# Snowdar/asv-subtools

Measured on AMD Instinct MI355X. Metric: utterances/sec (200-frame) embedding extraction + EER, 1/2/4/8 MI355X, higher is better.
Workload: dtype bf16; 1 GPU; BASELINE configs[1]: standard TDNN x-vector: Xvector(80,10,training=False), 80-dim fbank, 256 utterances x 200 frames per GPU per step, features resident in HBM, f32 embeddings out; global_batch_utts=256, frames_per_utt=200, parallelism=utterance shards x1, streams=2

## Files before the change

asv-subtools_amd/csrc/kernels_tdnn_p8.hip:

```cpp
#include <algorithm>
#include <cstdlib>
#include <type_traits>

#define ASV_GLDS_CLOBBER_M0
#include "lds_dma.h"

namespace asv {
namespace {

constexpr int P8_HALF = 128 * 128;
constexpr int P8_OFF_B0 = 0, P8_OFF_A0 = P8_HALF, P8_OFF_B1 = 2 * P8_HALF, P8_OFF_A1 = 3 * P8_HALF;
constexpr int P8_BUF = 4 * P8_HALF;
constexpr int P8_PARAM_OFF = 2 * P8_BUF;
constexpr int P8_LDS_BYTES = 2 * P8_BUF + 3 * 256 * 4;
constexpr int P8_ROWB = 128;

template <int ET, int VAR, bool ONE_TAP, int PH>
__global__ __launch_bounds__(512, 2) void tdnn_gemm_p8_kernel(const TdnnKernelParams p, int m_tiles, int n_tiles) {
  static_assert(PH == 2 || PH == 4, "phases per K-tile");
  constexpr bool STAGGER = !(VAR == 1 || VAR == 3), PRIO = !(VAR == 2 || VAR == 3), SKELETON = VAR == 4;
  constexpr bool NO_DMA = SKELETON || VAR == 5, NO_READS = SKELETON || VAR == 6;
  auto stamp = [&](int k) {
    if constexpr (VAR == 7) {
      if (threadIdx.x == 0) reinterpret_cast<unsigned long long *>(p.partial)[(size_t)blockIdx.x * 8 + k] = __builtin_amdgcn_s_memtime();
    }
  };
  stamp(0);
  __shared__ __attribute__((aligned(16))) unsigned char lds[P8_LDS_BYTES];
  const int tid = threadIdx.x, lane = tid & 63;
  const int wave = __builtin_amdgcn_readfirstlane(tid >> 6);
  const int wm = wave >> 2, wn = wave & 3;
  const int lr = lane & 31, lh = lane >> 5;

  const int tile = xcd_swizzle(blockIdx.x, m_tiles * n_tiles);
  const int m0 = (tile / n_tiles) * 256;
  const int n0 = (tile % n_tiles) * 256;

  const unsigned char *xg = reinterpret_cast<const unsigned char *>(p.x);
  const unsigned char *wg = reinterpret_cast<const unsigned char *>(p.w);
  const uint32_t x_pitch = (uint32_t)p.ldx * 2u;
  const int cin_pad = p.cin_pad;
  const int n_taps = ONE_TAP ? 1 : p.n_taps;
  const uint32_t w_pitch = (uint32_t)n_taps * (uint32_t)cin_pad * 2u;
  const uint32_t lds_base = __builtin_amdgcn_readfirstlane((uint32_t)(uintptr_t)(lds_byte *)lds);
  const int nkt = (cin_pad / 64) * n_taps;

  float *lds_par = reinterpret_cast<float *>(lds + P8_PARAM_OFF);
  auto stage_params = [&]() {
    if (wave < 3) {
      const float *src = (wave == 0) ? p.bias : (wave == 1 ? p.scale : p.shift);
      if (src != nullptr) {
        glds16_s_m0(src + n0, (uint32_t)lane * 16u, __builtin_amdgcn_readfirstlane(lds_base + (uint32_t)P8_PARAM_OFF + (uint32_t)wave * 1024u));
      } else {
        const float dflt = (wave == 1) ? 1.0f : 0.0f;
        *reinterpret_cast<float4 *>(lds_par + wave * 256 + lane * 4) = make_float4(dflt, dflt, dflt, dflt);
      }
    }
  };

  const int g_row = lane >> 3, g_slot = lane & 7;
  int a_row[2];
  uint32_t a_slot[2];
  uint32_t a_voff[2][2];
  uint32_t b_off[2];
  const int last_row = p.rows - 1;
#pragma unroll
  for (int i = 0; i < 2; ++i) {
    const int r = (wave * 2 + i) * 8 + g_row;
    const uint32_t slot16 = (uint32_t)(g_slot ^ ((r >> 1) & 7)) * 16u;
    a_row[i] = m0 + (r >> 6) * 128 + (r & 63);
    a_slot[i] = slot16;
    a_voff[0][i] = (uint32_t)a_row[i] * x_pitch + slot16;
    a_voff[1][i] = (uint32_t)min(a_row[i] + 64, last_row) * x_pitch + slot16;
    b_off[i] = (uint32_t)(n0 + (r >> 5) * 64 + (r & 31)) * w_pitch + slot16;
  }
  int v_taps = p.taps[0];
  if (!ONE_TAP) {
#pragma unroll
    for (int t = 1; t < ASV_MAX_TAPS; ++t) v_taps = (lane == t) ? p.taps[t] : v_taps;
  }

  auto stage = [&](int which, int c, int t, int b, bool in_loop) {
    if (NO_DMA && in_loop) return;
    const uint32_t dst0 = lds_base + (uint32_t)b * P8_BUF + (uint32_t)which * P8_HALF + (uint32_t)wave * 2048u;
    if (which & 1) {
      const unsigned char *base = xg + (size_t)c * 128;
      if (ONE_TAP) {
#pragma unroll
        for (int i = 0; i < 2; ++i) glds16_s_m0(base, a_voff[which == 3][i], __builtin_amdgcn_readfirstlane(dst0 + i * 1024u));
      } else {
        const int d = __builtin_amdgcn_readlane(v_taps, t) + (which == 3 ? 64 : 0);
#pragma unroll
        for (int i = 0; i < 2; ++i) {
          const int row = min(max(a_row[i] + d, 0), last_row);
          glds16_s_m0(base, (uint32_t)row * x_pitch + a_slot[i], __builtin_amdgcn_readfirstlane(dst0 + i * 1024u));
        }
      }
    } else {
      const unsigned char *base = wg + ((size_t)t * cin_pad + (size_t)c * 64) * 2 + (which == 2 ? (size_t)32 * w_pitch : 0);
#pragma unroll
      for (int i = 0; i < 2; ++i) glds16_s_m0(base, b_off[i], __builtin_amdgcn_readfirstlane(dst0 + i * 1024u));
    }
  };

  const uint32_t sw = (uint32_t)((lr >> 1) & 7);
  const uint32_t a_base = (uint32_t)(wm * 64 + lr) * P8_ROWB, b_base = (uint32_t)(wn * 32 + lr) * P8_ROWB;
  uint32_t a_addr[4], b_addr[4];
#pragma unroll
  for (int kg = 0; kg < 4; ++kg) {
    const uint32_t s16 = (((uint32_t)(kg * 2 + lh)) ^ sw) * 16u;
    a_addr[kg] = a_base + s16;
    b_addr[kg] = b_base + s16;
  }

  f32x16_t acc[4][2];
#pragma unroll
  for (int i = 0; i < 4; ++i)
#pragma unroll
    for (int j = 0; j < 2; ++j)
#pragma unroll
      for (int r = 0; r < 16; ++r) acc[i][j][r] = 0.0f;

  if constexpr (PH == 2) {
    stage_params();
    stage(0, 0, 0, 0, false); stage(1, 0, 0, 0, false); stage(2, 0, 0, 0, false); stage(3, 0, 0, 0, false);
    {
      int c1 = 0, t1 = 1;
      if (t1 == n_taps) { t1 = 0; c1 = 1; }
      if (nkt > 1) {
        stage(0, c1, t1, 1, false); stage(1, c1, t1, 1, false);
        asm volatile("s_waitcnt vmcnt(4)" ::: "memory");
      } else {
        asm volatile("s_waitcnt vmcnt(0)" ::: "memory");
      }
    }
    __builtin_amdgcn_s_barrier();
    asm volatile("" ::: "memory");
    uint4 wb0[4], wb1[4], xa[2][4];
    if (NO_READS) {
#pragma unroll
      for (int kg = 0; kg < 4; ++kg) {
        wb0[kg] = make_uint4(lane, 1, 2, 3); wb1[kg] = make_uint4(3, lane, 1, 0);
        xa[0][kg] = make_uint4(1, 1, lane, 1); xa[1][kg] = make_uint4(2, 2, 2, lane);
      }
    }
    stamp(1);
    if (STAGGER && wm == 1) __builtin_amdgcn_s_barrier();
    auto mma_q = [&](const uint4 (&wfr)[4], int j, int i0) {
#pragma unroll
      for (int kg = 0; kg < 4; ++kg)
#pragma unroll
        for (int i2 = 0; i2 < 2; ++i2) acc[i0 + i2][j] = mfma16<ET>(wfr[kg], xa[i2][kg], acc[i0 + i2][j]);
    };
    auto barrier = [&]() {
      __builtin_amdgcn_s_barrier();
      asm volatile("" ::: "memory");
    };
    int c1 = 0, t1 = 0, c2 = 0, t2 = 0;
    auto adv = [&](int &c, int &t) { if (++t == n_taps) { t = 0; ++c; } };
    adv(c1, t1); adv(c2, t2); adv(c2, t2);
    auto ktile2 = [&](int kt, auto tail_c) {
      constexpr int TAIL = decltype(tail_c)::value;
      const int b = kt & 1;
      const unsigned char *L = lds + (uint32_t)b * P8_BUF;
      if (!NO_READS) {
#pragma unroll
        for (int kg = 0; kg < 4; ++kg) wb0[kg] = *reinterpret_cast<const uint4 *>(L + P8_OFF_B0 + b_addr[kg]);
#pragma unroll
        for (int kg = 0; kg < 4; ++kg)
#pragma unroll
          for (int i2 = 0; i2 < 2; ++i2) xa[i2][kg] = *reinterpret_cast<const uint4 *>(L + P8_OFF_A0 + i2 * (32 * P8_ROWB) + a_addr[kg]);
#pragma unroll
        for (int kg = 0; kg < 4; ++kg) wb1[kg] = *reinterpret_cast<const uint4 *>(L + P8_OFF_B1 + b_addr[kg]);
        __builtin_amdgcn_sched_barrier(0);
      }
      if (TAIL <= 1) { stage(2, c1, t1, b ^ 1, true); stage(3, c1, t1, b ^ 1, true); }
      if (TAIL <= 1) asm volatile("s_waitcnt vmcnt(8) lgkmcnt(0)" ::: "memory");
      else asm volatile("s_waitcnt vmcnt(0) lgkmcnt(0)" ::: "memory");
      barrier();
      __builtin_amdgcn_sched_barrier(0);
      if (PRIO) __builtin_amdgcn_s_setprio(1);
      mma_q(wb0, 0, 0);
      mma_q(wb1, 1, 0);
      if (PRIO) __builtin_amdgcn_s_setprio(0);
      __builtin_amdgcn_sched_barrier(0);
      barrier();
      if (!NO_READS) {
#pragma unroll
        for (int kg = 0; kg < 4; ++kg)
#pragma unroll
          for (int i2 = 0; i2 < 2; ++i2) xa[i2][kg] = *reinterpret_cast<const uint4 *>(L + P8_OFF_A1 + i2 * (32 * P8_ROWB) + a_addr[kg]);
        __builtin_amdgcn_sched_barrier(0);
      }
      if (TAIL == 0) { stage(0, c2, t2, b, true); stage(1, c2, t2, b, true); }
      if (TAIL == 0) asm volatile("s_waitcnt vmcnt(6) lgkmcnt(0)" ::: "memory");
      else if (TAIL == 1) asm volatile("s_waitcnt vmcnt(2) lgkmcnt(0)" ::: "memory");
      else asm volatile("s_waitcnt lgkmcnt(0)" ::: "memory");
      barrier();
      __builtin_amdgcn_sched_barrier(0);
      if (PRIO) __builtin_amdgcn_s_setprio(1);
      mma_q(wb1, 1, 2);
      mma_q(wb0, 0, 2);
      if (PRIO) __builtin_amdgcn_s_setprio(0);
      __builtin_amdgcn_sched_barrier(0);
      barrier();
      adv(c1, t1); adv(c2, t2);
    };
    using J0 = std::integral_constant<int, 0>; using J1 = std::integral_constant<int, 1>; using J2 = std::integral_constant<int, 2>;
    int kt = 0;
    for (; kt + 2 < nkt; ++kt) ktile2(kt, J0{});
    if (kt + 1 < nkt) { ktile2(kt, J1{}); ++kt; }
    ktile2(kt, J2{});
  } else {
  {
    int c1 = 0, t1 = 1;
    if (t1 == n_taps) { t1 = 0; c1 = 1; }
    stage_params();
    stage(0, 0, 0, 0, false); stage(1, 0, 0, 0, false); stage(2, 0, 0, 0, false); stage(3, 0, 0, 0, false);
    if (nkt > 1) {
      stage(0, c1, t1, 1, false); stage(1, c1, t1, 1, false); stage(2, c1, t1, 1, false);
      asm volatile("s_waitcnt vmcnt(6)" ::: "memory");
    } else {
      asm volatile("s_waitcnt vmcnt(0)" ::: "memory");
    }
  }
  __builtin_amdgcn_s_barrier();
  asm volatile("" ::: "memory");

  uint4 wb0[2][4], wb1[4], xa[2][4];
  if (NO_READS) {
#pragma unroll
    for (int kg = 0; kg < 4; ++kg) {
      wb0[0][kg] = make_uint4(lane, 1, 2, 3); wb0[1][kg] = make_uint4(lane, 5, 2, 3); wb1[kg] = make_uint4(3, lane, 1, 0);
      xa[0][kg] = make_uint4(1, 1, lane, 1); xa[1][kg] = make_uint4(2, 2, 2, lane);
    }
  } else {
#pragma unroll
    for (int kg = 0; kg < 4; ++kg) wb0[0][kg] = *reinterpret_cast<const uint4 *>(lds + P8_OFF_B0 + b_addr[kg]);
  }
  if (STAGGER && wm == 1) __builtin_amdgcn_s_barrier();

  auto mma_q = [&](const uint4 (&wfr)[4], int j, int i0) {
    if (PRIO) __builtin_amdgcn_s_setprio(1);
#pragma unroll
    for (int kg = 0; kg < 4; ++kg)
#pragma unroll
      for (int i2 = 0; i2 < 2; ++i2) acc[i0 + i2][j] = mfma16<ET>(wfr[kg], xa[i2][kg], acc[i0 + i2][j]);
    if (PRIO) __builtin_amdgcn_s_setprio(0);
  };
  auto barrier = [&]() {
    __builtin_amdgcn_s_barrier();
    asm volatile("" ::: "memory");
  };

  int cs = 0, ts = 0;
  auto advance = [&]() { if (++ts == n_taps) { ts = 0; ++cs; } };
  advance();
  auto ktile = [&](auto tail_c, auto par_c) {
    constexpr int TAIL = decltype(tail_c)::value, PAR = decltype(par_c)::value;
    const unsigned char *L = lds + PAR * P8_BUF, *Ln = lds + (PAR ^ 1) * P8_BUF;
    if (!NO_READS) {
#pragma unroll
      for (int kg = 0; kg < 4; ++kg)
#pragma unroll
        for (int i2 = 0; i2 < 2; ++i2) xa[i2][kg] = *reinterpret_cast<const uint4 *>(L + P8_OFF_A0 + i2 * (32 * P8_ROWB) + a_addr[kg]);
      __builtin_amdgcn_sched_barrier(0);
    }
    if (TAIL <= 1) stage(3, cs, ts, PAR ^ 1, true);
    if (TAIL == 0) advance();
    barrier();
    asm volatile("s_waitcnt lgkmcnt(0)" ::: "memory");
    __builtin_amdgcn_sched_barrier(0);
    mma_q(wb0[PAR], 0, 0);
    __builtin_amdgcn_sched_barrier(0);
    barrier();
    if (!NO_READS) {
#pragma unroll
      for (int kg = 0; kg < 4; ++kg) wb1[kg] = *reinterpret_cast<const uint4 *>(L + P8_OFF_B1 + b_addr[kg]);
      __builtin_amdgcn_sched_barrier(0);
    }
    if (TAIL == 0) stage(0, cs, ts, PAR, true);
    barrier();
    asm volatile("s_waitcnt lgkmcnt(0)" ::: "memory");
    __builtin_amdgcn_sched_barrier(0);
    mma_q(wb1, 1, 0);
    __builtin_amdgcn_sched_barrier(0);
    barrier();
    if (!NO_READS) {
#pragma unroll
      for (int kg = 0; kg < 4; ++kg)
#pragma unroll
        for (int i2 = 0; i2 < 2; ++i2) xa[i2][kg] = *reinterpret_cast<const uint4 *>(L + P8_OFF_A1 + i2 * (32 * P8_ROWB) + a_addr[kg]);
      __builtin_amdgcn_sched_barrier(0);
    }
    if (TAIL == 0) {
      stage(1, cs, ts, PAR, true);
      asm volatile("s_waitcnt vmcnt(10)" ::: "memory");
    } else if (TAIL == 1) {
      asm volatile("s_waitcnt vmcnt(6)" ::: "memory");
    }
    barrier();
    asm volatile("s_waitcnt lgkmcnt(0)" ::: "memory");
    __builtin_amdgcn_sched_barrier(0);
    mma_q(wb1, 1, 2);
    __builtin_amdgcn_sched_barrier(0);
    barrier();
    if (!NO_READS && TAIL <= 1) {
#pragma unroll
      for (int kg = 0; kg < 4; ++kg) wb0[PAR ^ 1][kg] = *reinterpret_cast<const uint4 *>(Ln + P8_OFF_B0 + b_addr[kg]);
      __builtin_amdgcn_sched_barrier(0);
    }
    if (TAIL == 0) {
      stage(2, cs, ts, PAR, true);
      asm volatile("s_waitcnt vmcnt(6)" ::: "memory");
    } else if (TAIL == 1) {
      asm volatile("s_waitcnt vmcnt(0)" ::: "memory");
    }
    barrier();
    asm volatile("s_waitcnt lgkmcnt(0)" ::: "memory");
    __builtin_amdgcn_sched_barrier(0);
    mma_q(wb0[PAR], 0, 2);
    __builtin_amdgcn_sched_barrier(0);
    barrier();
  };
  using I0 = std::integral_constant<int, 0>; using I1 = std::integral_constant<int, 1>; using I2 = std::integral_constant<int, 2>;
  for (int kt = 0; kt + 2 < nkt; kt += 2) { ktile(I0{}, I0{}); ktile(I0{}, I1{}); }
  ktile(I1{}, I0{});
  ktile(I2{}, I1{});
  }
  if (STAGGER && wm == 0) __builtin_amdgcn_s_barrier();
  asm volatile("" ::: "memory");
  stamp(2);

  unsigned char *scr = lds + wave * (128 * P8_ROWB);
  const float act_lo = (p.act1 == ASV_ACT_RELU) ? 0.0f : -INFINITY;
  uint32_t vmask = 0;
#pragma unroll
  for (int i = 0; i < 4; ++i) vmask |= ((p.row_valid[(m0 + wm * 128 + i * 32) >> 5] >> lr) & 1u) << i;
#pragma unroll
  for (int j = 0; j < 2; ++j) {
#pragma unroll
    for (int q = 0; q < 4; ++q) {
      const int chl = wn * 64 + j * 32 + 8 * q + 4 * lh;
      const float4 b4 = *reinterpret_cast<const float4 *>(lds_par + chl);
      const float4 sc4 = *reinterpret_cast<const float4 *>(lds_par + 256 + chl);
      const float4 sh4 = *reinterpret_cast<const float4 *>(lds_par + 512 + chl);
      const float b[4] = {b4.x, b4.y, b4.z, b4.w}, sc[4] = {sc4.x, sc4.y, sc4.z, sc4.w}, sh[4] = {sh4.x, sh4.y, sh4.z, sh4.w};
      const int slot = j * 4 + q;
#pragma unroll
      for (int i = 0; i < 4; ++i) {
        const bool valid = (vmask >> i) & 1u;
        const int frow = i * 32 + lr;
        float y[4];
#pragma unroll
        for (int e = 0; e < 4; ++e) y[e] = tdnn_epilogue_fast(acc[i][j][q * 4 + e], b[e], act_lo, sc[e], sh[e], true);
        uint2 pk;
        pk.x = pack_h16x2<ET>(y[0], y[1]);
        pk.y = pack_h16x2<ET>(y[2], y[3]);
        pk.x = valid ? pk.x : 0u;
        pk.y = valid ? pk.y : 0u;
        *reinterpret_cast<uint2 *>(scr + frow * P8_ROWB + lds_swz(frow, slot) * 16 + ((lh ^ (frow & 1)) * 8)) = pk;
      }
    }
  }
  {
    unsigned char *yg = reinterpret_cast<unsigned char *>(p.y);
    const size_t y_pitch = (size_t)p.ldy * 2;
#pragma unroll
    for (int it = 0; it < 16; ++it) {
      const int piece = it * 64 + lane, frow = piece >> 3, slot = piece & 7;
      uint4 v = *reinterpret_cast<const uint4 *>(scr + frow * P8_ROWB + lds_swz(frow, slot) * 16);
      if (frow & 1) v = make_uint4(v.z, v.w, v.x, v.y);
      const int ch = n0 + wn * 64 + slot * 8;
      const int row = m0 + wm * 128 + frow;
      if (ch < p.cout_store) *reinterpret_cast<uint4 *>(yg + (size_t)row * y_pitch + (size_t)ch * 2) = v;
    }
  }
  if constexpr (VAR == 7) {
    asm volatile("s_waitcnt vmcnt(0)" ::: "memory");
    stamp(3);
  }
}


constexpr int P8P_PAR_SLOT = 4096;
constexpr int P8P_LDS_BYTES = 2 * P8_BUF + 2 * P8P_PAR_SLOT;

template <int ET, bool ONE_TAP>
__global__ __launch_bounds__(512, 2) void tdnn_gemm_p8p_kernel(const TdnnKernelParams p, int m_tiles, int n_tiles) {
  __shared__ __attribute__((aligned(16))) unsigned char lds[P8P_LDS_BYTES];
  const int tid = threadIdx.x, lane = tid & 63;
  const int wave = __builtin_amdgcn_readfirstlane(tid >> 6);
  const int wm = wave >> 2, wn = wave & 3;
  const int lr = lane & 31, lh = lane >> 5;
  const int total = m_tiles * n_tiles;
  const int grid = gridDim.x;

  const unsigned char *xg = reinterpret_cast<const unsigned char *>(p.x);
  const unsigned char *wg = reinterpret_cast<const unsigned char *>(p.w);
  const uint32_t x_pitch = (uint32_t)p.ldx * 2u;
  const int cin_pad = p.cin_pad;
  const int n_taps = ONE_TAP ? 1 : p.n_taps;
  const uint32_t w_pitch = (uint32_t)n_taps * (uint32_t)cin_pad * 2u;
  const uint32_t lds_base = __builtin_amdgcn_readfirstlane((uint32_t)(uintptr_t)(lds_byte *)lds);
  const int nkt = (cin_pad / 64) * n_taps;
  const int last_row = p.rows - 1;
  const int g_row = lane >> 3, g_slot = lane & 7;

  struct TileAddr { int m0, n0; int a_row[2]; uint32_t a_slot[2], a_voff[2][2], b_off[2]; };
  auto tile_addr = [&](int it) {
    TileAddr t;
    const int tile = xcd_swizzle(it, total);
    t.m0 = (tile / n_tiles) * 256;
    t.n0 = (tile % n_tiles) * 256;
#pragma unroll
    for (int i = 0; i < 2; ++i) {
      const int r = (wave * 2 + i) * 8 + g_row;
      const uint32_t slot16 = (uint32_t)(g_slot ^ ((r >> 1) & 7)) * 16u;
      t.a_row[i] = t.m0 + (r >> 6) * 128 + (r & 63);
      t.a_slot[i] = slot16;
      t.a_voff[0][i] = (uint32_t)t.a_row[i] * x_pitch + slot16;
      t.a_voff[1][i] = (uint32_t)min(t.a_row[i] + 64, last_row) * x_pitch + slot16;
      t.b_off[i] = (uint32_t)(t.n0 + (r >> 5) * 64 + (r & 31)) * w_pitch + slot16;
    }
    return t;
  };
  int v_taps = p.taps[0];
  if (!ONE_TAP) {
#pragma unroll
    for (int t = 1; t < ASV_MAX_TAPS; ++t) v_taps = (lane == t) ? p.taps[t] : v_taps;
  }
  auto stage = [&](const TileAddr &T, int which, int c, int t, int b) {
    const uint32_t dst0 = lds_base + (uint32_t)b * P8_BUF + (uint32_t)which * P8_HALF + (uint32_t)wave * 2048u;
    if (which & 1) {
      const unsigned char *base = xg + (size_t)c * 128;
      if (ONE_TAP) {
#pragma unroll
        for (int i = 0; i < 2; ++i) glds16_s_m0(base, T.a_voff[which == 3][i], __builtin_amdgcn_readfirstlane(dst0 + i * 1024u));
      } else {
        const int d = __builtin_amdgcn_readlane(v_taps, t) + (which == 3 ? 64 : 0);
#pragma unroll
        for (int i = 0; i < 2; ++i) {
          const int row = min(max(T.a_row[i] + d, 0), last_row);
          glds16_s_m0(base, (uint32_t)row * x_pitch + T.a_slot[i], __builtin_amdgcn_readfirstlane(dst0 + i * 1024u));
        }
      }
    } else {
      const unsigned char *base = wg + ((size_t)t * cin_pad + (size_t)c * 64) * 2 + (which == 2 ? (size_t)32 * w_pitch : 0);
#pragma unroll
      for (int i = 0; i < 2; ++i) glds16_s_m0(base, T.b_off[i], __builtin_amdgcn_readfirstlane(dst0 + i * 1024u));
    }
  };
  auto stage_tile_params = [&](const TileAddr &T, int slot) {
    const uint32_t dst = lds_base + 2u * P8_BUF + (uint32_t)slot * P8P_PAR_SLOT + (uint32_t)wave * 1024u;
    if (wave < 3) {
      const float *src = (wave == 0) ? p.bias : (wave == 1 ? p.scale : p.shift);
      if (src != nullptr) {
        glds16_s_m0(src + T.n0, (uint32_t)lane * 16u, __builtin_amdgcn_readfirstlane(dst));
      } else {
        const float dflt = (wave == 1) ? 1.0f : 0.0f;
        *reinterpret_cast<float4 *>(lds + 2 * P8_BUF + slot * P8P_PAR_SLOT + wave * 1024 + lane * 16) = make_float4(dflt, dflt, dflt, dflt);
      }
    } else if (wave == 3) {
      glds16_s_m0(p.row_valid + (T.m0 >> 5), lane < 2 ? (uint32_t)lane * 16u : 0u, __builtin_amdgcn_readfirstlane(dst));
    }
  };

  const uint32_t sw = (uint32_t)((lr >> 1) & 7);
  const uint32_t a_base = (uint32_t)(wm * 64 + lr) * P8_ROWB, b_base = (uint32_t)(wn * 32 + lr) * P8_ROWB;
  uint32_t a_addr[4], b_addr[4];
#pragma unroll
  for (int kg = 0; kg < 4; ++kg) {
    const uint32_t s16 = (((uint32_t)(kg * 2 + lh)) ^ sw) * 16u;
    a_addr[kg] = a_base + s16;
    b_addr[kg] = b_base + s16;
  }
  auto barrier = [&]() {
    __builtin_amdgcn_s_barrier();
    asm volatile("" ::: "memory");
  };
  auto kt_ct = [&](int kt, int &c, int &t) { c = kt / n_taps; t = kt - c * n_taps; };
  const float act_lo = (p.act1 == ASV_ACT_RELU) ? 0.0f : -INFINITY;
  unsigned char *yg = reinterpret_cast<unsigned char *>(p.y);
  const size_t y_pitch = (size_t)p.ldy * 2;

  int it = blockIdx.x;
  int slot = 0;
  TileAddr cur = tile_addr(it);
  stage_tile_params(cur, 0);
  stage(cur, 0, 0, 0, 0); stage(cur, 1, 0, 0, 0); stage(cur, 2, 0, 0, 0); stage(cur, 3, 0, 0, 0);
  if (nkt > 1) {
    int c1, t1;
    kt_ct(1, c1, t1);
    stage(cur, 0, c1, t1, 1); stage(cur, 1, c1, t1, 1);
  }
#pragma unroll 1
  while (true) {
    if (nkt > 1) asm volatile("s_waitcnt vmcnt(4)" ::: "memory");
    else asm volatile("s_waitcnt vmcnt(0)" ::: "memory");
    barrier();
    f32x16_t acc[4][2];
#pragma unroll
    for (int i = 0; i < 4; ++i)
#pragma unroll
      for (int j = 0; j < 2; ++j)
#pragma unroll
        for (int r = 0; r < 16; ++r) acc[i][j][r] = 0.0f;
    uint4 wb0[4], wb1[4], xa[2][4];
    if (wm == 1) __builtin_amdgcn_s_barrier();
    auto mma_q = [&](const uint4 (&wfr)[4], int j, int i0) {
#pragma unroll
      for (int kg = 0; kg < 4; ++kg)
#pragma unroll
        for (int i2 = 0; i2 < 2; ++i2) acc[i0 + i2][j] = mfma16<ET>(wfr[kg], xa[i2][kg], acc[i0 + i2][j]);
    };
    int c1 = 0, t1 = 0, c2 = 0, t2 = 0;
    auto adv = [&](int &c, int &t) { if (++t == n_taps) { t = 0; ++c; } };
    adv(c1, t1); adv(c2, t2); adv(c2, t2);
    auto ktile2 = [&](int kt, auto tail_c) {
      constexpr int TAIL = decltype(tail_c)::value;
      const int b = kt & 1;
      const unsigned char *L = lds + (uint32_t)b * P8_BUF;
#pragma unroll
      for (int kg = 0; kg < 4; ++kg) wb0[kg] = *reinterpret_cast<const uint4 *>(L + P8_OFF_B0 + b_addr[kg]);
#pragma unroll
      for (int kg = 0; kg < 4; ++kg)
#pragma unroll
        for (int i2 = 0; i2 < 2; ++i2) xa[i2][kg] = *reinterpret_cast<const uint4 *>(L + P8_OFF_A0 + i2 * (32 * P8_ROWB) + a_addr[kg]);
#pragma unroll
      for (int kg = 0; kg < 4; ++kg) wb1[kg] = *reinterpret_cast<const uint4 *>(L + P8_OFF_B1 + b_addr[kg]);
      __builtin_amdgcn_sched_barrier(0);
      if (TAIL <= 1) { stage(cur, 2, c1, t1, b ^ 1); stage(cur, 3, c1, t1, b ^ 1); }
      if (TAIL <= 1) asm volatile("s_waitcnt vmcnt(8) lgkmcnt(0)" ::: "memory");
      else asm volatile("s_waitcnt vmcnt(0) lgkmcnt(0)" ::: "memory");
      barrier();
      __builtin_amdgcn_sched_barrier(0);
      __builtin_amdgcn_s_setprio(1);
      mma_q(wb0, 0, 0);
      mma_q(wb1, 1, 0);
      __builtin_amdgcn_s_setprio(0);
      __builtin_amdgcn_sched_barrier(0);
      barrier();
#pragma unroll
      for (int kg = 0; kg < 4; ++kg)
#pragma unroll
        for (int i2 = 0; i2 < 2; ++i2) xa[i2][kg] = *reinterpret_cast<const uint4 *>(L + P8_OFF_A1 + i2 * (32 * P8_ROWB) + a_addr[kg]);
      __builtin_amdgcn_sched_barrier(0);
      if (TAIL == 0) { stage(cur, 0, c2, t2, b); stage(cur, 1, c2, t2, b); }
      if (TAIL == 0) asm volatile("s_waitcnt vmcnt(6) lgkmcnt(0)" ::: "memory");
      else if (TAIL == 1) asm volatile("s_waitcnt vmcnt(2) lgkmcnt(0)" ::: "memory");
      else asm volatile("s_waitcnt lgkmcnt(0)" ::: "memory");
      barrier();
      __builtin_amdgcn_sched_barrier(0);
      __builtin_amdgcn_s_setprio(1);
      mma_q(wb1, 1, 2);
      mma_q(wb0, 0, 2);
      __builtin_amdgcn_s_setprio(0);
      __builtin_amdgcn_sched_barrier(0);
      barrier();
      adv(c1, t1); adv(c2, t2);
    };
    using J0 = std::integral_constant<int, 0>; using J1 = std::integral_constant<int, 1>; using J2 = std::integral_constant<int, 2>;
    int kt = 0;
    for (; kt + 2 < nkt; ++kt) ktile2(kt, J0{});
    if (kt + 1 < nkt) { ktile2(kt, J1{}); ++kt; }
    ktile2(kt, J2{});
    if (wm == 0) __builtin_amdgcn_s_barrier();
    asm volatile("" ::: "memory");

    const bool has_next = it + grid < total;
    TileAddr nxt = cur;
    if (has_next) {
      nxt = tile_addr(it + grid);
      stage_tile_params(nxt, slot ^ 1);
      stage(nxt, 0, 0, 0, 0); stage(nxt, 1, 0, 0, 0); stage(nxt, 2, 0, 0, 0); stage(nxt, 3, 0, 0, 0);
    }
    {
      const float *par = reinterpret_cast<const float *>(lds + 2 * P8_BUF + slot * P8P_PAR_SLOT);
      const uint32_t *vw = reinterpret_cast<const uint32_t *>(lds + 2 * P8_BUF + slot * P8P_PAR_SLOT + 3072);
      unsigned char *scr = lds + P8_BUF + wave * (64 * P8_ROWB);
#pragma unroll
      for (int h = 0; h < 2; ++h) {
        uint32_t vmask = 0;
#pragma unroll
        for (int i2 = 0; i2 < 2; ++i2) vmask |= ((vw[wm * 4 + h * 2 + i2] >> lr) & 1u) << i2;
#pragma unroll
        for (int j = 0; j < 2; ++j) {
#pragma unroll
          for (int q = 0; q < 4; ++q) {
            const int chl = wn * 64 + j * 32 + 8 * q + 4 * lh;
            const float4 b4 = *reinterpret_cast<const float4 *>(par + chl);
            const float4 sc4 = *reinterpret_cast<const float4 *>(par + 256 + chl);
            const float4 sh4 = *reinterpret_cast<const float4 *>(par + 512 + chl);
            const float b[4] = {b4.x, b4.y, b4.z, b4.w}, sc[4] = {sc4.x, sc4.y, sc4.z, sc4.w}, sh[4] = {sh4.x, sh4.y, sh4.z, sh4.w};
            const int sl = j * 4 + q;
#pragma unroll
            for (int i2 = 0; i2 < 2; ++i2) {
              const bool valid = (vmask >> i2) & 1u;
              const int frow = i2 * 32 + lr;
              float y[4];
#pragma unroll
              for (int e = 0; e < 4; ++e) y[e] = tdnn_epilogue_fast(acc[h * 2 + i2][j][q * 4 + e], b[e], act_lo, sc[e], sh[e], true);
              uint2 pk;
              pk.x = pack_h16x2<ET>(y[0], y[1]);
              pk.y = pack_h16x2<ET>(y[2], y[3]);
              pk.x = valid ? pk.x : 0u;
              pk.y = valid ? pk.y : 0u;
              *reinterpret_cast<uint2 *>(scr + frow * P8_ROWB + lds_swz(frow, sl) * 16 + ((lh ^ (frow & 1)) * 8)) = pk;
            }
          }
        }
#pragma unroll
        for (int s8 = 0; s8 < 8; ++s8) {
          const int piece = s8 * 64 + lane, frow = piece >> 3, sl = piece & 7;
          uint4 v = *reinterpret_cast<const uint4 *>(scr + frow * P8_ROWB + lds_swz(frow, sl) * 16);
          if (frow & 1) v = make_uint4(v.z, v.w, v.x, v.y);
          const int ch = cur.n0 + wn * 64 + sl * 8;
          const int row = cur.m0 + wm * 128 + h * 64 + frow;
          if (ch < p.cout_store) *reinterpret_cast<uint4 *>(yg + (size_t)row * y_pitch + (size_t)ch * 2) = v;
        }
      }
    }
    if (!has_next) break;
    barrier();
    if (nkt > 1) {
      int c1n, t1n;
      kt_ct(1, c1n, t1n);
      stage(nxt, 0, c1n, t1n, 1); stage(nxt, 1, c1n, t1n, 1);
    }
    cur = nxt;
    slot ^= 1;
    it += grid;
  }
}

}

bool tdnn_p8_supported(const TdnnKernelParams &p, int et, bool out_f32) {
  const bool fits32 = (unsigned long long)p.rows * (unsigned long long)p.ldx * 2ull < (1ull << 32) &&
                      (unsigned long long)round_up(p.cout_store, 256) * (unsigned long long)p.n_taps * (unsigned long long)p.cin_pad * 2ull < (1ull << 32);
  const bool fast = (p.act1 == ASV_ACT_NONE || p.act1 == ASV_ACT_RELU) && p.act2 == ASV_ACT_NONE && !p.affine_first;
  return p.w != nullptr && et != ET_F32 && !out_f32 && fits32 && fast && p.x2 == nullptr && p.seg_bias == nullptr && p.seg_scale == nullptr && p.res == nullptr &&
         p.pool_partial == nullptr && p.rows % 256 == 0 && p.rows >= 256 && p.cin_pad % 64 == 0 && p.cin_pad >= 64 && p.cout_store % 8 == 0 && p.cout_store >= 192 &&
         p.n_taps >= 1 && p.n_taps <= ASV_MAX_TAPS && p.row_valid != nullptr;
}

int launch_tdnn_p8_variant(const TdnnKernelParams &p, int variant, hipStream_t s) {
  ASV_REQUIRE(tdnn_p8_supported(p, p.et, false), "tdnn(p8): layer shape not supported (rows %d cin %d cout %d taps %d)", p.rows, p.cin_pad, p.cout_store, p.n_taps);
  const int m_tiles = p.rows / 256, n_tiles = round_up(p.cout_store, 256) / 256;
  const dim3 grid(m_tiles * n_tiles), block(512);
  const bool f16 = p.et == ET_F16;
  const bool one = p.n_taps == 1 && p.taps[0] == 0;
#define ASV_P8(ETV, VARV) ASV_P8P(ETV, VARV, 2)
#define ASV_P8P(ETV, VARV, PHV) do { if (one) hipLaunchKernelGGL((tdnn_gemm_p8_kernel<ETV, VARV, true, PHV>), grid, block, 0, s, p, m_tiles, n_tiles); \
                               else hipLaunchKernelGGL((tdnn_gemm_p8_kernel<ETV, VARV, false, PHV>), grid, block, 0, s, p, m_tiles, n_tiles); } while (0)
  switch (variant) {
#ifdef ASV_WITH_ABLATION
    case 1: ASV_P8(ET_BF16, 1); break;
    case 2: ASV_P8(ET_BF16, 2); break;
    case 4: ASV_P8(ET_BF16, 4); break;
    case 5: ASV_P8(ET_BF16, 5); break;
    case 6: ASV_P8(ET_BF16, 6); break;
    case 7: ASV_P8(ET_BF16, 7); break;
    case 40: case 41: case 44:
      ASV_REQUIRE(((p.cin_pad / 64) * p.n_taps) % 2 == 0, "tdnn(p8): the four-phase form takes an even number of K-tiles");
      if (variant == 40) ASV_P8P(ET_BF16, 0, 4); else if (variant == 41) ASV_P8P(ET_BF16, 1, 4); else ASV_P8P(ET_BF16, 4, 4);
      break;
#endif
    case 50:
      if (f16) ASV_P8(ET_F16, 0);
      else ASV_P8(ET_BF16, 0);
      break;
    default: {
      static int cus = 0;
      if (cus == 0) {
        int dev = 0, n = 256;
        if (hipGetDevice(&dev) == hipSuccess) (void)hipDeviceGetAttribute(&n, hipDeviceAttributeMultiprocessorCount, dev);
        cus = n > 0 ? n : 256;
      }
      const dim3 pgrid(std::min(m_tiles * n_tiles, cus));
      if (one) { if (f16) hipLaunchKernelGGL((tdnn_gemm_p8p_kernel<ET_F16, true>), pgrid, block, 0, s, p, m_tiles, n_tiles);
                 else hipLaunchKernelGGL((tdnn_gemm_p8p_kernel<ET_BF16, true>), pgrid, block, 0, s, p, m_tiles, n_tiles); }
      else { if (f16) hipLaunchKernelGGL((tdnn_gemm_p8p_kernel<ET_F16, false>), pgrid, block, 0, s, p, m_tiles, n_tiles);
             else hipLaunchKernelGGL((tdnn_gemm_p8p_kernel<ET_BF16, false>), pgrid, block, 0, s, p, m_tiles, n_tiles); }
    }
  }
#undef ASV_P8
#undef ASV_P8P
  ASV_HIP_CHECK(hipGetLastError());
  return ASV_OK;
}

int launch_tdnn_p8(const TdnnKernelParams &p, hipStream_t s) { return launch_tdnn_p8_variant(p, 0, s); }

}
```

Measured before the change: 995,900 utterances/s.

## Switch persistent TDNN GEMM to 16x16 MFMA shape by default

Adds a NARROW template path to the persistent p8p TDNN GEMM kernel that uses 16x16 MFMA tiles (f32x4 accumulators) instead of 32x32, with matching LDS fragment reads and a reworked epilogue mapping. It is enabled by default through P8_MFMA_NARROW. The one-tap A-tile offset is also simplified to a base-pointer shift, which drops one per-tile address array and saves registers. The narrow shape may change LDS read patterns and MFMA throughput, and it adds timing-stamp and ablation variants.

```diff
diff --git a/asv-subtools_amd/csrc/kernels_tdnn_p8.hip b/asv-subtools_amd/csrc/kernels_tdnn_p8.hip
--- a/asv-subtools_amd/csrc/kernels_tdnn_p8.hip
+++ b/asv-subtools_amd/csrc/kernels_tdnn_p8.hip
@@ -386,13 +386,18 @@
 constexpr int P8P_PAR_SLOT = 4096;
 constexpr int P8P_LDS_BYTES = 2 * P8_BUF + 2 * P8P_PAR_SLOT;
 
-template <int ET, bool ONE_TAP>
+template <int ET, bool ONE_TAP, bool NARROW, bool STAMP = false>
 __global__ __launch_bounds__(512, 2) void tdnn_gemm_p8p_kernel(const TdnnKernelParams p, int m_tiles, int n_tiles) {
   __shared__ __attribute__((aligned(16))) unsigned char lds[P8P_LDS_BYTES];
   const int tid = threadIdx.x, lane = tid & 63;
   const int wave = __builtin_amdgcn_readfirstlane(tid >> 6);
   const int wm = wave >> 2, wn = wave & 3;
-  const int lr = lane & 31, lh = lane >> 5;
+  const int lr = NARROW ? (lane & 15) : (lane & 31), lh = NARROW ? (lane >> 4) : (lane >> 5);
+  auto stamp = [&](int k) {
+    if constexpr (STAMP) {
+      if (tid == 0) reinterpret_cast<unsigned long long *>(p.partial)[(size_t)blockIdx.x * 8 + k] = __builtin_amdgcn_s_memtime();
+    }
+  };
   const int total = m_tiles * n_tiles;
   const int grid = gridDim.x;
 
@@ -407,7 +412,7 @@
   const int last_row = p.rows - 1;
   const int g_row = lane >> 3, g_slot = lane & 7;
 
-  struct TileAddr { int m0, n0; int a_row[2]; uint32_t a_slot[2], a_voff[2][2], b_off[2]; };
+  struct TileAddr { int m0, n0; int a_row[2]; uint32_t a_slot[2], a_voff[2], b_off[2]; };
   auto tile_addr = [&](int it) {
     TileAddr t;
     const int tile = xcd_swizzle(it, total);
@@ -419,8 +424,7 @@
       const uint32_t slot16 = (uint32_t)(g_slot ^ ((r >> 1) & 7)) * 16u;
       t.a_row[i] = t.m0 + (r >> 6) * 128 + (r & 63);
       t.a_slot[i] = slot16;
-      t.a_voff[0][i] = (uint32_t)t.a_row[i] * x_pitch + slot16;
-      t.a_voff[1][i] = (uint32_t)min(t.a_row[i] + 64, last_row) * x_pitch + slot16;
+      t.a_voff[i] = (uint32_t)t.a_row[i] * x_pitch + slot16;
       t.b_off[i] = (uint32_t)(t.n0 + (r >> 5) * 64 + (r & 31)) * w_pitch + slot16;
     }
     return t;
@@ -435,8 +439,9 @@
     if (which & 1) {
       const unsigned char *base = xg + (size_t)c * 128;
       if (ONE_TAP) {
-#pragma unroll
-        for (int i = 0; i < 2; ++i) glds16_s_m0(base, T.a_voff[which == 3][i], __builtin_amdgcn_readfirstlane(dst0 + i * 1024u));
+        const unsigned char *base1 = base + (which == 3 ? (size_t)64 * x_pitch : 0);
+#pragma unroll
+        for (int i = 0; i < 2; ++i) glds16_s_m0(base1, T.a_voff[i], __builtin_amdgcn_readfirstlane(dst0 + i * 1024u));
       } else {
         const int d = __builtin_amdgcn_readlane(v_taps, t) + (which == 3 ? 64 : 0);
 #pragma unroll
@@ -471,13 +476,37 @@
   uint32_t a_addr[4], b_addr[4];
 #pragma unroll
   for (int kg = 0; kg < 4; ++kg) {
-    const uint32_t s16 = (((uint32_t)(kg * 2 + lh)) ^ sw) * 16u;
+    const uint32_t s16 = (((uint32_t)(NARROW ? kg * 4 + lh : kg * 2 + lh)) ^ sw) * 16u;
     a_addr[kg] = a_base + s16;
     b_addr[kg] = b_base + s16;
   }
   auto barrier = [&]() {
     __builtin_amdgcn_s_barrier();
     asm volatile("" ::: "memory");
+  };
+  auto read_b = [&](const unsigned char *H, uint4 (&wfr)[4]) {
+    if constexpr (NARROW) {
+#pragma unroll
+      for (int ks = 0; ks < 2; ++ks)
+#pragma unroll
+        for (int c2 = 0; c2 < 2; ++c2) wfr[ks * 2 + c2] = *reinterpret_cast<const uint4 *>(H + c2 * (16 * P8_ROWB) + b_addr[ks]);
+    } else {
+#pragma unroll
+      for (int kg = 0; kg < 4; ++kg) wfr[kg] = *reinterpret_cast<const uint4 *>(H + b_addr[kg]);
+    }
+  };
+  auto read_a = [&](const unsigned char *H, uint4 (&xa)[8]) {
+    if constexpr (NARROW) {
+#pragma unroll
+      for (int f4 = 0; f4 < 4; ++f4)
+#pragma unroll
+        for (int ks = 0; ks < 2; ++ks) xa[f4 * 2 + ks] = *reinterpret_cast<const uint4 *>(H + f4 * (16 * P8_ROWB) + a_addr[ks]);
+    } else {
+#pragma unroll
+      for (int kg = 0; kg < 4; ++kg)
+#pragma unroll
+        for (int i2 = 0; i2 < 2; ++i2) xa[i2 * 4 + kg] = *reinterpret_cast<const uint4 *>(H + i2 * (32 * P8_ROWB) + a_addr[kg]);
+    }
   };
   auto kt_ct = [&](int kt, int &c, int &t) { c = kt / n_taps; t = kt - c * n_taps; };
   const float act_lo = (p.act1 == ASV_ACT_RELU) ? 0.0f : -INFINITY;
@@ -500,19 +529,40 @@
     else asm volatile("s_waitcnt vmcnt(0)" ::: "memory");
     barrier();
     f32x16_t acc[4][2];
-#pragma unroll
-    for (int i = 0; i < 4; ++i)
-#pragma unroll
-      for (int j = 0; j < 2; ++j)
-#pragma unroll
-        for (int r = 0; r < 16; ++r) acc[i][j][r] = 0.0f;
-    uint4 wb0[4], wb1[4], xa[2][4];
+    f32x4_t accn[8][4];
+    if constexpr (NARROW) {
+#pragma unroll
+      for (int f = 0; f < 8; ++f)
+#pragma unroll
+        for (int cf = 0; cf < 4; ++cf)
+#pragma unroll
+          for (int r = 0; r < 4; ++r) accn[f][cf][r] = 0.0f;
+    } else {
+#pragma unroll
+      for (int i = 0; i < 4; ++i)
+#pragma unroll
+        for (int j = 0; j < 2; ++j)
+#pragma unroll
+          for (int r = 0; r < 16; ++r) acc[i][j][r] = 0.0f;
+    }
+    uint4 wb0[4], wb1[4], xa[8];
+    if (it == (int)blockIdx.x) stamp(1);
     if (wm == 1) __builtin_amdgcn_s_barrier();
     auto mma_q = [&](const uint4 (&wfr)[4], int j, int i0) {
-#pragma unroll
-      for (int kg = 0; kg < 4; ++kg)
-#pragma unroll
-        for (int i2 = 0; i2 < 2; ++i2) acc[i0 + i2][j] = mfma16<ET>(wfr[kg], xa[i2][kg], acc[i0 + i2][j]);
+      if constexpr (NARROW) {
+#pragma unroll
+        for (int ks = 0; ks < 2; ++ks)
+#pragma unroll
+          for (int f4 = 0; f4 < 4; ++f4)
+#pragma unroll
+            for (int c2 = 0; c2 < 2; ++c2)
+              accn[i0 * 2 + f4][j * 2 + c2] = mfma16n<ET>(wfr[ks * 2 + c2], xa[f4 * 2 + ks], accn[i0 * 2 + f4][j * 2 + c2]);
+      } else {
+#pragma unroll
+        for (int kg = 0; kg < 4; ++kg)
+#pragma unroll
+          for (int i2 = 0; i2 < 2; ++i2) acc[i0 + i2][j] = mfma16<ET>(wfr[kg], xa[i2 * 4 + kg], acc[i0 + i2][j]);
+      }
     };
     int c1 = 0, t1 = 0, c2 = 0, t2 = 0;
     auto adv = [&](int &c, int &t) { if (++t == n_taps) { t = 0; ++c; } };
@@ -521,14 +571,9 @@
       constexpr int TAIL = decltype(tail_c)::value;
       const int b = kt & 1;
       const unsigned char *L = lds + (uint32_t)b * P8_BUF;
-#pragma unroll
-      for (int kg = 0; kg < 4; ++kg) wb0[kg] = *reinterpret_cast<const uint4 *>(L + P8_OFF_B0 + b_addr[kg]);
-#pragma unroll
-      for (int kg = 0; kg < 4; ++kg)
-#pragma unroll
-        for (int i2 = 0; i2 < 2; ++i2) xa[i2][kg] = *reinterpret_cast<const uint4 *>(L + P8_OFF_A0 + i2 * (32 * P8_ROWB) + a_addr[kg]);
-#pragma unroll
-      for (int kg = 0; kg < 4; ++kg) wb1[kg] = *reinterpret_cast<const uint4 *>(L + P8_OFF_B1 + b_addr[kg]);
+      read_b(L + P8_OFF_B0, wb0);
+      read_a(L + P8_OFF_A0, xa);
+      read_b(L + P8_OFF_B1, wb1);
       __builtin_amdgcn_sched_barrier(0);
       if (TAIL <= 1) { stage(cur, 2, c1, t1, b ^ 1); stage(cur, 3, c1, t1, b ^ 1); }
       if (TAIL <= 1) asm volatile("s_waitcnt vmcnt(8) lgkmcnt(0)" ::: "memory");
@@ -541,10 +586,7 @@
       __builtin_amdgcn_s_setprio(0);
       __builtin_amdgcn_sched_barrier(0);
       barrier();
-#pragma unroll
-      for (int kg = 0; kg < 4; ++kg)
-#pragma unroll
-        for (int i2 = 0; i2 < 2; ++i2) xa[i2][kg] = *reinterpret_cast<const uint4 *>(L + P8_OFF_A1 + i2 * (32 * P8_ROWB) + a_addr[kg]);
+      read_a(L + P8_OFF_A1, xa);
       __builtin_amdgcn_sched_barrier(0);
       if (TAIL == 0) { stage(cur, 0, c2, t2, b); stage(cur, 1, c2, t2, b); }
       if (TAIL == 0) asm volatile("s_waitcnt vmcnt(6) lgkmcnt(0)" ::: "memory");
@@ -567,6 +609,7 @@
     ktile2(kt, J2{});
     if (wm == 0) __builtin_amdgcn_s_barrier();
     asm volatile("" ::: "memory");
+    if (it == (int)blockIdx.x) stamp(2);
 
     const bool has_next = it + grid < total;
     TileAddr nxt = cur;
@@ -581,32 +624,61 @@
       unsigned char *scr = lds + P8_BUF + wave * (64 * P8_ROWB);
 #pragma unroll
       for (int h = 0; h < 2; ++h) {
-        uint32_t vmask = 0;
-#pragma unroll
-        for (int i2 = 0; i2 < 2; ++i2) vmask |= ((vw[wm * 4 + h * 2 + i2] >> lr) & 1u) << i2;
-#pragma unroll
-        for (int j = 0; j < 2; ++j) {
-#pragma unroll
-          for (int q = 0; q < 4; ++q) {
-            const int chl = wn * 64 + j * 32 + 8 * q + 4 * lh;
+        if constexpr (NARROW) {
+          uint32_t vmask = 0;
+#pragma unroll
+          for (int f4 = 0; f4 < 4; ++f4) vmask |= ((vw[wm * 4 + h * 2 + (f4 >> 1)] >> ((f4 & 1) * 16 + lr)) & 1u) << f4;
+#pragma unroll
+          for (int cf = 0; cf < 4; ++cf) {
+            const int chl = wn * 64 + cf * 16 + 4 * lh;
             const float4 b4 = *reinterpret_cast<const float4 *>(par + chl);
             const float4 sc4 = *reinterpret_cast<const float4 *>(par + 256 + chl);
             const float4 sh4 = *reinterpret_cast<const float4 *>(par + 512 + chl);
             const float b[4] = {b4.x, b4.y, b4.z, b4.w}, sc[4] = {sc4.x, sc4.y, sc4.z, sc4.w}, sh[4] = {sh4.x, sh4.y, sh4.z, sh4.w};
-            const int sl = j * 4 + q;
-#pragma unroll
-            for (int i2 = 0; i2 < 2; ++i2) {
-              const bool valid = (vmask >> i2) & 1u;
-              const int frow = i2 * 32 + lr;
+            const int sl = cf * 2 + (lh >> 1);
+#pragma unroll
+            for (int f4 = 0; f4 < 4; ++f4) {
+              const bool valid = (vmask >> f4) & 1u;
+              const int frow = f4 * 16 + lr;
               float y[4];
 #pragma unroll
-              for (int e = 0; e < 4; ++e) y[e] = tdnn_epilogue_fast(acc[h * 2 + i2][j][q * 4 + e], b[e], act_lo, sc[e], sh[e], true);
+              for (int e = 0; e < 4; ++e) y[e] = tdnn_epilogue_fast(accn[h * 4 + f4][cf][e], b[e], act_lo, sc[e], sh[e], true);
               uint2 pk;
               pk.x = pack_h16x2<ET>(y[0], y[1]);
               pk.y = pack_h16x2<ET>(y[2], y[3]);
               pk.x = valid ? pk.x : 0u;
               pk.y = valid ? pk.y : 0u;
-              *reinterpret_cast<uint2 *>(scr + frow * P8_ROWB + lds_swz(frow, sl) * 16 + ((lh ^ (frow & 1)) * 8)) = pk;
+              *reinterpret_cast<uint2 *>(scr + frow * P8_ROWB + lds_swz(frow, sl) * 16 + (((lh & 1) ^ (frow & 1)) * 8)) = pk;
+            }
+          }
+        } else {
+          uint32_t vmask = 0;
+#pragma unroll
+          for (int i2 = 0; i2 < 2; ++i2) vmask |= ((vw[wm * 4 + h * 2 + i2] >> lr) & 1u) << i2;
+#pragma unroll
+          for (int j = 0; j < 2; ++j) {
+#pragma unroll
+            for (int q = 0; q < 4; ++q) {
+              const int chl = wn * 64 + j * 32 + 8 * q + 4 * lh;
+              const float4 b4 = *reinterpret_cast<const float4 *>(par + chl);
+              const float4 sc4 = *reinterpret_cast<const float4 *>(par + 256 + chl);
+              const float4 sh4 = *reinterpret_cast<const float4 *>(par + 512 + chl);
+              const float b[4] = {b4.x, b4.y, b4.z, b4.w}, sc[4] = {sc4.x, sc4.y, sc4.z, sc4.w}, sh[4] = {sh4.x, sh4.y, sh4.z, sh4.w};
+              const int sl = j * 4 + q;
+#pragma unroll
+              for (int i2 = 0; i2 < 2; ++i2) {
+                const bool valid = (vmask >> i2) & 1u;
+                const int frow = i2 * 32 + lr;
+                float y[4];
+#pragma unroll
+                for (int e = 0; e < 4; ++e) y[e] = tdnn_epilogue_fast(acc[h * 2 + i2][j][q * 4 + e], b[e], act_lo, sc[e], sh[e], true);
+                uint2 pk;
+                pk.x = pack_h16x2<ET>(y[0], y[1]);
+                pk.y = pack_h16x2<ET>(y[2], y[3]);
+                pk.x = valid ? pk.x : 0u;
+                pk.y = valid ? pk.y : 0u;
+                *reinterpret_cast<uint2 *>(scr + frow * P8_ROWB + lds_swz(frow, sl) * 16 + ((lh ^ (frow & 1)) * 8)) = pk;
+              }
             }
           }
         }
@@ -632,6 +704,21 @@
     slot ^= 1;
     it += grid;
   }
+}
+
+#ifndef P8_MFMA_NARROW
+#define P8_MFMA_NARROW 1
+#endif
+constexpr bool kP8Narrow = P8_MFMA_NARROW != 0;
+
+template <bool NARROW>
+void launch_p8p(const TdnnKernelParams &p, bool one, dim3 grid, int m_tiles, int n_tiles, hipStream_t s) {
+  const dim3 block(512);
+  const bool f16 = p.et == ET_F16;
+  if (one) { if (f16) hipLaunchKernelGGL((tdnn_gemm_p8p_kernel<ET_F16, true, NARROW>), grid, block, 0, s, p, m_tiles, n_tiles);
+             else hipLaunchKernelGGL((tdnn_gemm_p8p_kernel<ET_BF16, true, NARROW>), grid, block, 0, s, p, m_tiles, n_tiles); }
+  else { if (f16) hipLaunchKernelGGL((tdnn_gemm_p8p_kernel<ET_F16, false, NARROW>), grid, block, 0, s, p, m_tiles, n_tiles);
+         else hipLaunchKernelGGL((tdnn_gemm_p8p_kernel<ET_BF16, false, NARROW>), grid, block, 0, s, p, m_tiles, n_tiles); }
 }
 
 }
@@ -679,10 +766,25 @@
         cus = n > 0 ? n : 256;
       }
       const dim3 pgrid(std::min(m_tiles * n_tiles, cus));
-      if (one) { if (f16) hipLaunchKernelGGL((tdnn_gemm_p8p_kernel<ET_F16, true>), pgrid, block, 0, s, p, m_tiles, n_tiles);
-                 else hipLaunchKernelGGL((tdnn_gemm_p8p_kernel<ET_BF16, true>), pgrid, block, 0, s, p, m_tiles, n_tiles); }
-      else { if (f16) hipLaunchKernelGGL((tdnn_gemm_p8p_kernel<ET_F16, false>), pgrid, block, 0, s, p, m_tiles, n_tiles);
-             else hipLaunchKernelGGL((tdnn_gemm_p8p_kernel<ET_BF16, false>), pgrid, block, 0, s, p, m_tiles, n_tiles); }
+#ifdef ASV_WITH_ABLATION
+      static const bool live = getenv("ASV_AMD_LIVE_TUNE") != nullptr;
+      auto read_int = [](const char *name) { const char *v = getenv(name); return v != nullptr ? atoi(v) : -1; };
+      static const int mfma0 = read_int("ASV_AMD_P8_MFMA");
+      int shape = live ? read_int("ASV_AMD_P8_MFMA") : mfma0;
+      if (variant == 60 || variant == 62) shape = 0;
+      if (variant == 61 || variant == 63) shape = 1;
+      if (variant == 62 || variant == 63) {
+        ASV_REQUIRE(!f16 && p.partial != nullptr, "tdnn(p8): the stamped forms are bf16 and write p.partial");
+        if (variant == 62) { if (one) hipLaunchKernelGGL((tdnn_gemm_p8p_kernel<ET_BF16, true, false, true>), pgrid, block, 0, s, p, m_tiles, n_tiles);
+                             else hipLaunchKernelGGL((tdnn_gemm_p8p_kernel<ET_BF16, false, false, true>), pgrid, block, 0, s, p, m_tiles, n_tiles); }
+        else { if (one) hipLaunchKernelGGL((tdnn_gemm_p8p_kernel<ET_BF16, true, true, true>), pgrid, block, 0, s, p, m_tiles, n_tiles);
+               else hipLaunchKernelGGL((tdnn_gemm_p8p_kernel<ET_BF16, false, true, true>), pgrid, block, 0, s, p, m_tiles, n_tiles); }
+        break;
+      }
+      if (shape == 0) { launch_p8p<false>(p, one, pgrid, m_tiles, n_tiles, s); break; }
+      if (shape == 1) { launch_p8p<true>(p, one, pgrid, m_tiles, n_tiles, s); break; }
+#endif
+      launch_p8p<kP8Narrow>(p, one, pgrid, m_tiles, n_tiles, s);
     }
   }
 #undef ASV_P8
```

After: 1.012 million utterances/s (median of 6 runs). 1.02x the previous value.
